# emma-mens/adam-compression

Hardware: AMD Instinct MI355X
Metric: grad elements/s per DGC step (HBM GB/s % of peak), 0.1% ratio, 1-8 GPUs (higher is better)
Workload: dtype f32

## Files before the change

adam-compression_amd/csrc/select.hip:

```cpp
#include <algorithm>
#include <cstdlib>
#include <cstring>
#include <cmath>
#include <vector>

#include "radix_select.hpp"
#include "introselect.hpp"

namespace dgc {

constexpr int kSeg = 1024;
constexpr int kCap = 64;
constexpr int kLstTile = 4;
__host__ __device__ __forceinline__ int64_t lcol(int64_t seg) {
    return (seg / kLstTile) * (kLstTile * kCap) + seg % kLstTile;
}
__host__ __device__ __forceinline__ int64_t lslot(int64_t seg, int64_t e, int64_t ntile) {
    (void)ntile;
    return lcol(seg) + e * kLstTile;
}
constexpr int kSegTiles = kSeg / (kWave * 4);
constexpr int kSuper = 4;
constexpr int kGroupSegs = 1024;
constexpr int kCountSegs = 4;
// ... 1330 lines not shown
    uint32_t vs[kSegTiles];
    load_segment(vec, d.n, ls, xs, vs);
    emit_segment_firstk(xs, vs, d, ls, base, limit, obase, t, o, mask_now);
}


constexpr int kEmitSegs = kGroupSegs / kEmitSplit;
constexpr int kEmitBatch = 16;
constexpr int kEmitShort = 16;
constexpr uint32_t kEmitSkip = 0xFFFFFFFFu;
static_assert(kCap == kWave, "wave-per-list emission needs kCap == wavefront width");

__device__ __forceinline__ void emit_body(const float* __restrict__ vec_flat, const SelWS& w, const EmitOut& oa,
                                          int64_t bx) {
    const int t = task(w, BT_GRP, (int)bx);
    const SelState* st = w.st + t;
    if (st->branch == DGC_BRANCH_RESAMPLE && st->rs_nth == 2) return;
    if (st->spec_emitted) return;
    const bool k5 = st->branch == DGC_BRANCH_RESAMPLE && st->rs_nth == 1;
    if (k5 && !oa.queue) return;
    EmitOut o = oa;
    if (!k5) o.queue = nullptr;
    const TDesc d = w.td[t];
    const bool defer_here = o.defer && !k5 && !d.tail;
    const float* vec = vec_flat + d.off;
    const int64_t lb = bx - w.bt[BT_GRP][t];
    const int64_t lg = lb / kEmitSplit;
    const int sub = (int)(lb % kEmitSplit);
    const int64_t g = d.grp0 + lg;
    const int64_t lseg0 = lg * kGroupSegs + (int64_t)sub * kEmitSegs;
    __shared__ uint32_t off_a[kEmitSegs], lcn[kEmitSegs];
    __shared__ uint64_t lds16[16];
    __shared__ long long obase_s;
    if (threadIdx.x < kWave) {
        const long long b = k5 ? 0 : out_base(w, t);
        if (threadIdx.x == 0) obase_s = b;
    }
    const long long limit = k5 ? st->n_cur : st->limit;
    const long long ga = w.grp_off[g];
    const float tc = st->t_cur;
    {
        const int jq = (int)threadIdx.x;
        const int64_t ls = lseg0 + jq;
        uint32_t ca = 0, lc = 0, pa = 0;
        if (ls < d.nseg) {
            const int64_t seg = d.seg0 + ls;
            ca = w.seg_cnt[seg];
            lc = lcnt_count(w.seg_lcnt[seg]);
        }
#pragma unroll
        for (int q = 0; q < kEmitSplit - 1; ++q) {
            if (q < sub) {
                const int64_t seg = d.seg0 + lg * kGroupSegs + (int64_t)q * kEmitSegs + threadIdx.x;
                pa += w.seg_cnt[seg];
            }
        }
        const bool short_list = ls < d.nseg && ca > 0 && lc <= (uint32_t)kEmitShort;
        float v[kEmitShort];
        uint16_t e[kEmitShort];
        if (short_list) {
            const int64_t ntile = ceil_div(w.nseg, (int64_t)kLstTile);
#pragma unroll
            for (int q = 0; q < kEmitShort; ++q)
                if ((uint32_t)q < lc) {
                    v[q] = w.lst_val[lslot(d.seg0 + ls, q, ntile)];
                    e[q] = w.lst_off[lslot(d.seg0 + ls, q, ntile)];
                }
        }
        uint64_t tot;
        const uint64_t ra = block_exclusive_scan(((uint64_t)pa << 32) | ca, lds16, &tot);
        const uint32_t oa = (uint32_t)(tot >> 32) + (uint32_t)ra;
        const bool work = ca > 0 && ga + oa < limit;
        if (defer_here && ls < d.nseg) w.seg_off[d.seg0 + ls] = oa;
        off_a[jq] = oa;
        lcn[jq] = (work && !short_list) ? lc : kEmitSkip;
        __syncthreads();
        if (work && short_list) {
            const long long ob0 = obase_s;
            long long pos = ga + oa;
#pragma unroll
            for (int j = 0; j < kEmitShort; ++j)
                if ((uint32_t)j < lc && fabsf(v[j]) >= tc) {
                    if (pos < limit) emit_one(o, d, ob0 + pos, ls * kSeg + e[j], v[j], !defer_here);
                    ++pos;
                }
        }
    }
    __syncthreads();
    const long long obase = obase_s;
    const int lane = threadIdx.x & 63, wv = threadIdx.x >> 6;
    const uint64_t lt = lanemask_lt();
    constexpr int kWaveSegs = kEmitSegs / (kEmitSegs / kWave);
    const int jw = wv * kWaveSegs;
    const uint32_t Lme = lane < kWaveSegs ? lcn[jw + lane] : kEmitSkip;
    uint64_t todo = __ballot(Lme != kEmitSkip && Lme <= (uint32_t)kCap);
    uint64_t spilled = __ballot(Lme != kEmitSkip && Lme > (uint32_t)kCap);
    for (int b0 = 0; b0 < kWaveSegs; b0 += kEmitBatch) {
        if (!((todo >> b0) & ((1ull << kEmitBatch) - 1))) continue;
        const int j0 = jw + b0;
        float x[kEmitBatch];
        uint32_t e[kEmitBatch];
#pragma unroll
        for (int q = 0; q < kEmitBatch; ++q) {
            const uint32_t L = lcn[j0 + q];
            x[q] = 0.f;
            e[q] = 0;
            if (L <= (uint32_t)kCap && (uint32_t)lane < L) {
                const int64_t slot = lslot(d.seg0 + lseg0 + j0 + q, lane, ceil_div(w.nseg, (int64_t)kLstTile));
                x[q] = w.lst_val[slot];
                e[q] = w.lst_off[slot];
            }
        }
#pragma unroll
        for (int q = 0; q < kEmitBatch; ++q) {
            const uint32_t L = lcn[j0 + q];
            if (L == kEmitSkip || L > (uint32_t)kCap) continue;
            const int64_t ls = lseg0 + j0 + q;
            const long long ba = ga + off_a[j0 + q];
            const bool sel = (uint32_t)lane < L && fabsf(x[q]) >= tc;
            const uint64_t m = __ballot(sel);
            const long long pos = ba + __popcll(m & lt);
            if (sel && pos < limit) emit_one(o, d, obase + pos, ls * kSeg + e[q], x[q], !defer_here);
        }
    }
    while (spilled) {
        const int j = jw + __builtin_ctzll(spilled);
        spilled &= spilled - 1;
        emit_reread_firstk(vec, d, lseg0 + j, ga + off_a[j], limit, obase, tc, o, !defer_here);
    }
}

__global__ void __launch_bounds__(kEmitSegs)
k_emit(const float* __restrict__ vec_flat, SelWS w, EmitOut oa) {
    emit_body(vec_flat, w, oa, blockIdx.x);
}

constexpr int kChainPhases = 3;
enum { CH_CLAIM = 0, CH_GATE = kChainPhases };
static_assert(32 + kChainPhases * 32 <= kChainOneWords, "SelWS::chain words");

template <bool ALIGNED>
__global__ void __launch_bounds__(kBlock)
k_chain_one(const float* __restrict__ vec_flat, SelWS w, SelCfg p) {
    uint32_t* cc = w.chain;
    __shared__ uint32_t s_u;
    bool open = false;
    for (int t = threadIdx.x; !open && t < w.T; t += blockDim.x) open = !w.st[t].done;
    if (!__syncthreads_or(open)) return;
    for (int ph = 0; ph < kChainPhases; ++ph) {
        bool any = false;
        for (int t = threadIdx.x; !any && t < w.T; t += blockDim.x) {
            const SelState& u = w.st[t];
            any = ph < 2 ? u.lower_pending != 0 : (u.active && u.t_cur >= u.t_list);
        }
        any = __syncthreads_or(any);
        if (threadIdx.x == 0) {
            uint32_t gate = __hip_atomic_load(&cc[CH_GATE + ph], __ATOMIC_RELAXED, __HIP_MEMORY_SCOPE_AGENT);
            if (gate == 0) {
                const uint32_t want = any ? 2u : 1u;
                const uint32_t prev = atomicCAS(&cc[CH_GATE + ph], 0u, want);
                gate = prev == 0u ? want : prev;
            }
            s_u = gate;
        }
        __syncthreads();
        if (s_u != 2u) continue;
        const int which = ph == 0 ? BT_SEG : ph == 1 ? BT_CAP4 : BT_CNT;
        const uint32_t nvb = (uint32_t)w.bt[which][w.T];
        uint32_t mine = 0;
        for (;;) {
            __syncthreads();
            if (threadIdx.x == 0) s_u = atomicAdd(&cc[CH_CLAIM + ph], 1u);
            __syncthreads();
            const uint32_t vb = s_u;
            if (vb >= nvb) break;
            if (ph == 0) lower_lists_body(vec_flat, w, p, vb);
            else if (ph == 1) lower_counts_body<ALIGNED>(vec_flat, w, p, vb);
            else count_lists_body(vec_flat, w, p, vb);
            ++mine;
        }
        chain_phase_end(reinterpret_cast<ChainPhase*>(cc + 32) + ph, mine, nvb);
    }
}



__device__ __forceinline__ void resample_set_block(const float* __restrict__ vec_flat, const SelWS& w,
                                                   const EmitOut& o, int bx, bool wait);

__device__ __forceinline__ bool emit_wide_part(const float* __restrict__ vec_flat, const SelWS& w, const EmitOut& oa,
                                               int bx) {
    const int t = task(w, BT_GRP, bx);
    const SelState* st = w.st + t;
    if (st->branch == DGC_BRANCH_RESAMPLE && st->rs_nth == 2) return false;
    if (st->spec_emitted) return false;
    const bool k5 = st->branch == DGC_BRANCH_RESAMPLE && st->rs_nth == 1;
    if (k5 && !oa.queue) return false;
    EmitOut o = oa;
    if (!k5) o.queue = nullptr;
    const TDesc d = w.td[t];
    const bool defer_here = o.defer && !k5 && !d.tail;
    const float* vec = vec_flat + d.off;
    const int64_t lb = (int64_t)bx - w.bt[BT_GRP][t];
    constexpr int split = kEmitSplit;
    const int64_t lg = lb / split;
    const int sub = (int)(lb % split);
    const int64_t g = d.grp0 + lg;
    const int64_t lseg0 = lg * kGroupSegs;
    __shared__ uint32_t off_a[kGroupSegs], lcn[kGroupSegs];
    __shared__ uint64_t lds16[16];
    __shared__ long long obase_s;
    if (threadIdx.x < kWave) {
        const long long b = k5 ? 0 : out_base(w, t);
        if (threadIdx.x == 0) obase_s = b;
    }
    const long long limit = k5 ? st->n_cur : st->limit;
    const long long ga = w.grp_off[g];
    {
        const int64_t ls = lseg0 + threadIdx.x;
        uint32_t ca = 0, lc = 0;
        if (ls < d.nseg) {
            const int64_t seg = d.seg0 + ls;
            ca = w.seg_cnt[seg];
            lc = lcnt_count(w.seg_lcnt[seg]);
        }
        uint64_t tot;
        const uint32_t oa = (uint32_t)block_exclusive_scan((uint64_t)ca, lds16, &tot);
        const bool work = ca > 0 && ga + oa < limit;
        if (defer_here && ls < d.nseg && (int)threadIdx.x / (kGroupSegs / split) == sub)
            w.seg_off[d.seg0 + ls] = oa;
        off_a[threadIdx.x] = oa;
        lcn[threadIdx.x] = work ? lc : kEmitSkip;
    }
    __syncthreads();
    ES_STAMP(1);
    const long long obase = obase_s;
    const float tc = st->t_cur;
    const int lane = threadIdx.x & 63, wv = threadIdx.x >> 6;
    const uint64_t lt = lanemask_lt();
    constexpr int wave_segs = kGroupSegs / split / (kGroupSegs / kWave);
    static_assert(wave_segs % kEmitBatch == 0, "whole batches per wave");
    const int jw = sub * (kGroupSegs / split) + wv * wave_segs;
    for (int j0 = jw; j0 < jw + wave_segs; j0 += kEmitBatch) {
        float x[kEmitBatch];
        uint32_t e[kEmitBatch];
#pragma unroll
        for (int q = 0; q < kEmitBatch; ++q) {
            const uint32_t L = lcn[j0 + q];
            x[q] = 0.f;
            e[q] = 0;
            if (L <= (uint32_t)kCap && (uint32_t)lane < L) {
                const int64_t slot = lslot(d.seg0 + lseg0 + j0 + q, lane, ceil_div(w.nseg, (int64_t)kLstTile));
                x[q] = w.lst_val[slot];
                e[q] = w.lst_off[slot];
            }
        }
        uint32_t spilled = 0;
#pragma unroll
        for (int q = 0; q < kEmitBatch; ++q) {
            const uint32_t L = lcn[j0 + q];
            if (L == kEmitSkip) continue;
            const int64_t ls = lseg0 + j0 + q;
            const long long ba = ga + off_a[j0 + q];
            if (L > (uint32_t)kCap) {
                spilled |= 1u << q;
                continue;
            }
            const bool sel = (uint32_t)lane < L && fabsf(x[q]) >= tc;
            const uint64_t m = __ballot(sel);
            const long long pos = ba + __popcll(m & lt);
            if (sel && pos < limit) emit_one(o, d, obase + pos, ls * kSeg + e[q], x[q], !defer_here);
        }
        while (spilled) {
            const int q = __builtin_ctz(spilled);
            spilled &= spilled - 1;
            emit_reread_firstk(vec, d, lseg0 + j0 + q, ga + off_a[j0 + q], limit, obase, tc, o, !defer_here);
        }
    }
    return k5;
}

template <bool SET>
__global__ void __launch_bounds__(kGroupSegs)
k_emit_wide_t(const float* __restrict__ vec_flat, SelWS w, EmitOut oa, EmitOut os, int32_t ngb) {
    const int bx = (int)blockIdx.x;
    ES_STAMP(0);
    if (SET && bx >= ngb) {
        resample_set_block(vec_flat, w, os, bx - ngb, true);
    } else if (emit_wide_part(vec_flat, w, oa, bx) && SET) {
        const int t = task(w, BT_GRP, bx);
        asm volatile("s_waitcnt vmcnt(0)" ::: "memory");
        __syncthreads();
        if (threadIdx.x == 0) {
            __builtin_amdgcn_fence(__ATOMIC_RELEASE, "agent");
            __hip_atomic_fetch_add(&w.setg[t].gathered, 1u, __ATOMIC_RELAXED, __HIP_MEMORY_SCOPE_AGENT);
        }
    }
    ES_STAMP(2);
}

constexpr unsigned long long kLbAgg = 1ull << 62, kLbPre = 1ull << 63, kLbVal = kLbAgg - 1;
constexpr int kLbSpin = 1 << 22;
constexpr int kCeStage = 2048;
#ifdef DGC_K5_PROF
__device__ unsigned long long g_ce_prof[2048][6];
#define CE_STAMP(i) do { if (threadIdx.x == 0 && lg < 2048) g_ce_prof[lg][i] = wall_clock64(); } while (0)
#else
#define CE_STAMP(i) do { } while (0)
#endif

__device__ __forceinline__ void count_emit_body(const float* __restrict__ vec_flat, const SelWS& w, const SelCfg& p,
                                                const EmitOut& o) {
    static_assert(kBlock * kCountSegs == kGroupSegs && kCountSegs == kLstTile, "k_count_emit layout");
    SelState* st = w.st;
    if (!st->active || !(st->t_cur >= st->t_list)) return;
    const TDesc d = w.td[0];
    const float* vec = vec_flat + d.off;
    const float tc = st->t_cur;
    const uint32_t tkey = abs_key(tc);
    const int tid = threadIdx.x, lane = tid & 63, wave = wave_id();
    __shared__ uint32_t lg_s;
    __shared__ int nspill;
    __shared__ int spill[kGroupSegs];
    __shared__ uint32_t spill_cnt[kGroupSegs];
    __shared__ uint64_t lds16[16];
    __shared__ unsigned long long prefix_s;
    __shared__ float stage_v[kCeStage];
    __shared__ uint32_t stage_i[kCeStage];
    if (tid == 0) {
        lg_s = atomicAdd(&st->ce_ticket, 1u);
        nspill = 0;
    }
    __syncthreads();
    const int64_t lg = lg_s;
    CE_STAMP(0);
    const int64_t ls0 = lg * kGroupSegs + kCountSegs * tid;
    const int64_t seg0 = d.seg0 + ls0;
    uint32_t n[kCountSegs], c[kCountSegs], lc[kCountSegs];
    if (ls0 + 3 < d.nseg) {
        const uint4 u = *reinterpret_cast<const uint4*>(w.seg_lcnt + seg0);
        lc[0] = u.x; lc[1] = u.y; lc[2] = u.z; lc[3] = u.w;
    } else {
#pragma unroll
        for (int q = 0; q < kCountSegs; ++q) lc[q] = ls0 + q < d.nseg ? w.seg_lcnt[seg0 + q] : 0u;
    }
#pragma unroll
    for (int q = 0; q < kCountSegs; ++q) {
        n[q] = ((lc[q] >> 16) << 16) <= tkey ? 0u : lcnt_count(lc[q]);
        c[q] = 0;
    }
    uint32_t nmax = 0;
#pragma unroll
    for (int q = 0; q < kCountSegs; ++q)
        if (n[q] <= (uint32_t)kCap) nmax = max(nmax, n[q]);
    constexpr int kFirst = 8;
    const int64_t ntile = ceil_div(w.nseg, (int64_t)kLstTile);
    const float* lv = w.lst_val;
    const uint16_t* lo = w.lst_off;
    float4 a[kFirst];
#pragma unroll
    for (int e = 0; e < kFirst; ++e)
        if ((uint32_t)e < nmax) a[e] = *reinterpret_cast<const float4*>(lv + lslot(seg0, e, ntile));
#pragma unroll
    for (int e = 0; e < kFirst; ++e) {
        const float x[4] = {a[e].x, a[e].y, a[e].z, a[e].w};
#pragma unroll
        for (int q = 0; q < kCountSegs; ++q) c[q] += (uint32_t)e < n[q] && n[q] <= (uint32_t)kCap && fabsf(x[q]) >= tc;
    }
    for (uint32_t e0 = kFirst; e0 < nmax; e0 += kFirst) {
        float4 b[kFirst];
#pragma unroll
        for (int e = 0; e < kFirst; ++e)
            if (e0 + e < nmax) b[e] = *reinterpret_cast<const float4*>(lv + lslot(seg0, e0 + e, ntile));
#pragma unroll
        for (int e = 0; e < kFirst; ++e) {
            if (e0 + e >= nmax) break;
            const float x[4] = {b[e].x, b[e].y, b[e].z, b[e].w};
#pragma unroll
            for (int q = 0; q < kCountSegs; ++q)
                c[q] += e0 + e < n[q] && n[q] <= (uint32_t)kCap && fabsf(x[q]) >= tc;
        }
    }
#pragma unroll
    for (int q = 0; q < kCountSegs; ++q)
        if (ls0 + q < d.nseg && n[q] > (uint32_t)kCap) spill[atomicAdd(&nspill, 1)] = kCountSegs * tid + q;
    __syncthreads();
    for (int i = wave; i < nspill; i += kBlock / kWave) {
        const int j = spill[i];
        const uint32_t cs = wave_count_segment(vec, d.n, lg * kGroupSegs + j, tc);
        if (lane == 0) spill_cnt[j] = cs;
    }
    __syncthreads();
#pragma unroll
    for (int q = 0; q < kCountSegs; ++q)
        if (ls0 + q < d.nseg && n[q] > (uint32_t)kCap) c[q] = spill_cnt[kCountSegs * tid + q];
    CE_STAMP(1);
    const uint32_t mine = c[0] + c[1] + c[2] + c[3];
    uint64_t total;
    const uint32_t tbase = (uint32_t)block_exclusive_scan((uint64_t)mine, lds16, &total);
    uint32_t off[kCountSegs];
    off[0] = tbase;
#pragma unroll
    for (int q = 1; q < kCountSegs; ++q) off[q] = off[q - 1] + c[q - 1];
#pragma unroll
    for (int q = 0; q < kCountSegs; ++q)
        if (ls0 + q < d.nseg) {
            w.seg_cnt[seg0 + q] = c[q];
            w.seg_off[seg0 + q] = off[q];
            if (n[q] > (uint32_t)kCap) spill_cnt[kCountSegs * tid + q] = off[q];
        }
    if (wave == 0) {
        unsigned long long* lb = w.grp_lb + d.grp0;
        if (lane == 0) {
            if (total) atomicAdd(&w.grp_cnt[d.grp0 + lg], (unsigned long long)total);
            __hip_atomic_store(&lb[lg], (lg == 0 ? kLbPre : kLbAgg) | total, __ATOMIC_RELAXED,
                               __HIP_MEMORY_SCOPE_AGENT);
        }
        unsigned long long prefix = 0;
        bool ok = true;
        int64_t j = lg - 1;
        int spin = 0;
        while (j >= 0) {
            const int64_t jj = j - lane;
            const unsigned long long v =
                jj >= 0 ? __hip_atomic_load(&lb[jj], __ATOMIC_RELAXED, __HIP_MEMORY_SCOPE_AGENT) : kLbPre;
            const uint64_t pre = __ballot((v & kLbPre) != 0), unready = __ballot(v == 0);
            const int first = pre ? __builtin_ctzll(pre) : kWave;
            const uint64_t need = first >= kWave - 1 ? ~0ull : ((2ull << first) - 1);
            if (unready & need) {
                if (++spin > kLbSpin) {
                    ok = false;
                    break;
                }
                __builtin_amdgcn_s_sleep(1);
                continue;
            }
            prefix += wave_sum(lane <= first ? (v & kLbVal) : 0ull);
            if (first < kWave) break;
            j -= kWave;
        }
        if (lane == 0) {
            if (lg > 0 && ok)
                __hip_atomic_store(&lb[lg], kLbPre | (prefix + total), __ATOMIC_RELAXED, __HIP_MEMORY_SCOPE_AGENT);
            if (!ok) atomicExch(&st->ce_fail, 1);
            prefix_s = ok ? prefix : ~0ull;
        }
    }
    __syncthreads();
    CE_STAMP(2);
    const unsigned long long P = prefix_s;
    const long long limit = d.k;
    const bool emit = P != ~0ull && (long long)P < limit;
    const bool staged = emit && nspill == 0 && total <= (uint64_t)kCeStage;
    if (emit) {
        for (uint32_t e0 = 0; e0 < nmax; e0 += kFirst) {
            if ((long long)(P + off[0]) >= limit) break;
            uint2 ob[kFirst];
            float4 vb[kFirst];
#pragma unroll
            for (int e = 0; e < kFirst; ++e)
                if (e0 + e < nmax) {
                    ob[e] = *reinterpret_cast<const uint2*>(lo + lslot(seg0, e0 + e, ntile));
                    vb[e] = *reinterpret_cast<const float4*>(lv + lslot(seg0, e0 + e, ntile));
                }
#pragma unroll
            for (int e = 0; e < kFirst; ++e) {
                if (e0 + e >= nmax) break;
                const float x[4] = {vb[e].x, vb[e].y, vb[e].z, vb[e].w};
                const uint32_t oo[4] = {ob[e].x & 0xFFFFu, ob[e].x >> 16, ob[e].y & 0xFFFFu, ob[e].y >> 16};
#pragma unroll
                for (int q = 0; q < kCountSegs; ++q)
                    if (e0 + e < n[q] && n[q] <= (uint32_t)kCap && fabsf(x[q]) >= tc) {
                        const uint32_t r = off[q];
                        if (staged) {
                            stage_v[r] = x[q];
                            stage_i[r] = (uint32_t)(kCountSegs * tid + q) * kSeg + oo[q];
                        } else if ((long long)(P + r) < limit) {
                            emit_one(o, d, (long long)(P + r), (ls0 + q) * kSeg + oo[q], x[q], false);
                        }
                        off[q] = r + 1;
                    }
            }
        }
    }
    if (emit && !staged)
        for (int i = wave; i < nspill; i += kBlock / kWave) {
            const int j = spill[i];
            emit_reread_firstk(vec, d, lg * kGroupSegs + j, (long long)(P + spill_cnt[j]), limit, 0, tc, o, false);
        }
    CE_STAMP(3);
    if (staged) {
        __syncthreads();
        const long long m = std::min<long long>((long long)total, limit - (long long)P);
        const int64_t gbase = lg * kGroupSegs * (int64_t)kSeg;
        for (long long i = tid; i < m; i += kBlock) {
            store_value(o.values, (long long)P + i, stage_v[i], o.vdtype);
            store_index(o.indices, (long long)P + i, d.idx_base + gbase + stage_i[i], o.idtype);
        }
    }
    CE_STAMP(4);
    if (last_block_arrival8(st->tk8, (uint32_t)lg, (uint32_t)(w.bt[BT_CNT][1] - w.bt[BT_CNT][0])))
        decide_tensor(w, p, 0, 1);
    CE_STAMP(5);
}

__global__ void __launch_bounds__(kBlock)
k_count_emit(const float* __restrict__ vec_flat, SelWS w, SelCfg p, EmitOut o) {
    count_emit_body(vec_flat, w, p, o);
}

template <bool ALIGNED>
__global__ void __launch_bounds__(kBlock)
k_count_emit_pass(const float* __restrict__ vec_flat, SelWS w, SelCfg p, EmitOut o, int which, int ncnt) {
    if ((int)blockIdx.x < ncnt)
        count_emit_body(vec_flat, w, p, o);
    else
        select_pass_body<ALIGNED>(vec_flat, w, which, p, (int64_t)blockIdx.x - ncnt);
}

struct FinishArgs {
    int64_t* count_out;
    dgc_select_info* info;
    float margin;
    int32_t defer, mask_mmt;
    int32_t on;
    int32_t* sink;
    uint32_t force;
    int64_t* order_out;
};

__device__ __forceinline__ void sel_finish_body(const SelWS& w, const FinishArgs& f) {
    int64_t* count_out = f.count_out;
    dgc_select_info* info = f.info;
    const float margin = f.margin;
    const int defer = f.defer, mask_mmt = f.mask_mmt;
    __shared__ unsigned long long total;
    __shared__ uint32_t broken, topk_order;
    if (threadIdx.x == 0) {
        total = 0;
        broken = 0;
        topk_order = 0;
    }
    __syncthreads();
    for (int t = threadIdx.x; t < w.T; t += blockDim.x) {
        SelState* st = w.st + t;
        struct {
            float t0, t_cur;
            int32_t branch, recounts, overflow, full_passes, list_spills, epoch, tie_rule, win_keys;
            long long n_cur, limit;
        } s;
        s.t0 = st->t0;
        s.t_cur = st->t_cur;
        s.branch = st->branch;
        s.recounts = st->recounts;
        s.overflow = st->overflow;
        s.full_passes = st->full_passes;
        s.list_spills = st->list_spills;
        s.epoch = st->epoch;
        s.tie_rule = st->tie_rule;
        s.win_keys = st->win_keys;
        s.n_cur = st->n_cur;
        s.limit = st->limit;
        const uint32_t wc = st->win_cnt[s.epoch & 1];
        const int64_t k = w.td[t].k;
        const bool tail = w.td[t].tail;
        const uint32_t status = w.nthg[t].status;
        float* spec = w.spec ? w.spec + kSpecWords * t : nullptr;
        const float used = spec ? spec[0] : __builtin_huge_valf();
        const float prev = spec ? spec[1] : __builtin_huge_valf();
        const uint32_t k5 = status | (s.branch == DGC_BRANCH_RESAMPLE ? f.force : 0u);
        if (k5 & DGC_K5_BROKEN) atomicOr(&broken, k5);
        if (s.branch == DGC_BRANCH_RESAMPLE && s.tie_rule == DGC_TIES_EXACT) atomicOr(&topk_order, 1u);
        const long long cnt = s.branch == DGC_BRANCH_RESAMPLE ? (long long)k : s.limit;
        atomicAdd(&total, (unsigned long long)cnt);
        st->epoch = s.epoch + 1;
        st->def_mode = (defer && s.branch != DGC_BRANCH_RESAMPLE && !tail && cnt > 0) ? 1 : 0;
        st->def_t = s.t_cur;
        st->def_limit = s.limit;
        st->def_mask_mmt = mask_mmt;
        if (info) {
            dgc_select_info& r = info[t];
            r.count = cnt;
            r.candidates = s.n_cur;
            r.threshold0 = s.t0;
            r.threshold = s.t_cur;
            r.branch = s.branch;
            r.recounts = s.recounts;
            r.overflow_segments = s.full_passes ? s.overflow : s.list_spills;
            r.full_passes = s.full_passes;
            r.tie_rule = s.tie_rule;
            r.window_keys = s.win_keys;
            r.k5_status = (int32_t)k5;
            r.list_threshold = used;
        }
        if (spec) {
            const float tc = s.t_cur;
            const bool finite = tc == tc && tc > 0.f && tc < __builtin_huge_valf();
            const float gr = fminf(fmaxf(2.f - prev / tc, 1.f), 1.5f);
            const float c0 = spec[4] < __builtin_huge_valf() ? spec[4] : fmaxf(margin, kSpecCeil0);
            const bool tried = used < __builtin_huge_valf() && tc > 0.f;
            const bool hit = tried && tc >= used;
            const float mcap = !tried ? c0
                                : hit ? fminf(c0 + kSpecCeilUp, fmaxf(margin, kSpecMarginMax))
                                      : fmaxf(c0 - kSpecCeilDown, margin);
            float m = margin;
            if (hit) m = fminf(fmaxf(1.05f * (used / tc), margin), mcap);
            spec[4] = mcap;
            spec[0] = finite ? tc * m * gr : __builtin_huge_valf();
            spec[1] = finite ? tc : __builtin_huge_valf();
            const float t0 = s.t0;
            const bool f0 = t0 == t0 && t0 > 0.f && t0 < __builtin_huge_valf();
            const float g0 = fminf(fmaxf(2.f - spec[3] / t0, 1.f), 1.5f);
            const float mw = wc > (uint32_t)kWinMax ? 0.985f : (s.win_keys > 0 ? 0.97f : 0.9f);
            spec[2] = f0 ? t0 * mw * g0 : __builtin_huge_valf();
            spec[3] = f0 ? t0 : __builtin_huge_valf();
        }
    }
    __syncthreads();
    if (threadIdx.x == 0 && count_out) *count_out = (int64_t)total;
    if (threadIdx.x == 0 && f.order_out) *f.order_out = topk_order ? 0 : (int64_t)DGC_ORDER_ASCENDING;
    if (threadIdx.x == 0 && broken && f.sink)
        __hip_atomic_store(f.sink, (int32_t)broken, __ATOMIC_RELAXED, __HIP_MEMORY_SCOPE_SYSTEM);
}

__global__ void k_sel_finish(SelWS w, FinishArgs f) { sel_finish_body(w, f); }

__global__ void __launch_bounds__(kBlock) k_emit_queue(const float* __restrict__ vec_flat, SelWS w, EmitOut o) {
    const int t = task(w, BT_QUEUE, blockIdx.x);
    const SelState* st = w.st + t;
    if (!(st->branch == DGC_BRANCH_RESAMPLE && st->rs_nth == 1)) return;
    const TDesc d = w.td[t];
    __shared__ long long obase_s;
    if (threadIdx.x < kWave) {
        const long long b = out_base(w, t);
        if (threadIdx.x == 0) obase_s = b;
    }
    __syncthreads();
    const int64_t q = ((int64_t)blockIdx.x - w.bt[BT_QUEUE][t]) * kQueuePerBlock + threadIdx.x;
    if (q >= d.k) return;
    const uint32_t j = (uint32_t)w.queue[d.cand_off + q];
    emit_one(o, d, obase_s + q, w.cand_idx[d.cand_off + j], w.cand_val[d.cand_off + j]);
}

constexpr int kHeapTop = 16383;
constexpr int kHeapChunk = kNthThreads * 4;
constexpr int kHeapSub = 5;
constexpr int kHeapKeyShift = 33;
constexpr uint64_t kHeapIdxMask = (1ull << kHeapKeyShift) - 1;
constexpr size_t kHeapSmemBytes = (size_t)(kHeapTop + 1 + kHeapChunk) * 8;
constexpr size_t kK5SmemBytes = kHeapSmemBytes > kNthSmemBytes ? kHeapSmemBytes : kNthSmemBytes;

__device__ __forceinline__ uint32_t hkey(uint64_t e) { return (uint32_t)(e >> kHeapKeyShift); }

struct HeapNodes {
    DGC_LDS uint64_t* l;
    DGC_GLB uint64_t* g;
    __device__ __forceinline__ uint64_t ld(int64_t i) const { return i < kHeapTop ? l[i] : g[i]; }
    __device__ __forceinline__ void st(int64_t i, uint64_t v) const {
        if (i < kHeapTop)
            l[i] = v;
        else
            g[i] = v;
    }
};

__device__ void heap_adjust1(const HeapNodes& h, int64_t hole, int64_t len, uint64_t v) {
    const int64_t top = hole;
    int64_t child = hole;
    while (child < (len - 1) / 2) {
        child = 2 * (child + 1);
        const uint64_t r = h.ld(child), l = h.ld(child - 1);
        uint64_t c = r;
        if (hkey(r) > hkey(l)) {
            child--;
            c = l;
        }
        h.st(hole, c);
        hole = child;
    }
    if ((len & 1) == 0 && child == (len - 2) / 2) {
        child = 2 * (child + 1);
        h.st(hole, h.ld(child - 1));
        hole = child - 1;
    }
    int64_t parent = (hole - 1) / 2;
    while (hole > top) {
        const uint64_t pv = h.ld(parent);
        if (!(hkey(pv) > hkey(v))) break;
        h.st(hole, pv);
        hole = parent;
        parent = (hole - 1) / 2;
    }
    h.st(hole, v);
}

__device__ __forceinline__ uint64_t readlane64(uint64_t x, int lane) {
    const uint32_t lo = (uint32_t)__builtin_amdgcn_readlane((int)(uint32_t)x, lane);
    const uint32_t hi = (uint32_t)__builtin_amdgcn_readlane((int)(uint32_t)(x >> 32), lane);
    return ((uint64_t)hi << 32) | lo;
}

__device__ uint64_t heap_replace_root(const HeapNodes& h, int64_t len, uint64_t v) {
    const int lane = threadIdx.x & 63;
    uint64_t pidx = 0, pval = 0;
    int m = 0;
    int64_t hole = 0;
    bool more = len > 1;
    while (more) {
        const int dl = 31 - __clz(lane + 2);
        const int64_t ol = (int64_t)(lane + 2) - (1ll << dl);
        const int64_t node = ((hole + 1) << dl) - 1 + ol;
        uint64_t val = 0;
        if (lane < 62 && node < len) val = h.ld(node);
        int64_t off = 0;
        for (int d = 1; d <= kHeapSub; ++d) {
            const int base = (1 << d) - 2;
            int64_t child;
            uint64_t cval;
            if (hole < (len - 1) / 2) {
                const uint64_t l = readlane64(val, base + (int)(2 * off));
                const uint64_t r = readlane64(val, base + (int)(2 * off) + 1);
                if (hkey(r) > hkey(l)) {
                    child = 2 * hole + 1;
                    cval = l;
                    off = 2 * off;
                } else {
                    child = 2 * hole + 2;
                    cval = r;
                    off = 2 * off + 1;
                }
            } else if ((len & 1) == 0 && hole == (len - 2) / 2) {
                child = 2 * hole + 1;
                cval = readlane64(val, base + (int)(2 * off));
                off = 2 * off;
                more = false;
            } else {
                more = false;
                break;
            }
            if (lane == m) {
                pidx = (uint64_t)child;
                pval = cval;
            }
            ++m;
            hole = child;
            if (!more) break;
        }
    }
    const uint64_t above = __ballot(lane < m && hkey(pval) > hkey(v));
    const int jm1 = above ? __builtin_ctzll(above) : m;
    const uint64_t up = (uint64_t)__shfl_up((long long)pidx, 1);
    const int64_t parent = lane == 0 ? 0 : (int64_t)up;
    if (lane < jm1)
        h.st(parent, pval);
    else if (lane == jm1)
        h.st(parent, v);
    __builtin_amdgcn_fence(__ATOMIC_RELEASE, "workgroup");
    __builtin_amdgcn_fence(__ATOMIC_ACQUIRE, "workgroup");
    return jm1 == 0 ? v : readlane64(pval, 0);
}

constexpr int kHeapAhead = 8;

__device__ __forceinline__ void heap_load(const float* vec, int64_t n, int64_t c0, bool al, float (&x)[4]) {
    const int64_t e0 = c0 + 4 * (int64_t)threadIdx.x;
    if (al && e0 + 3 < n) {
        const float4 v = *reinterpret_cast<const float4*>(vec + e0);
        x[0] = v.x;
        x[1] = v.y;
        x[2] = v.z;
        x[3] = v.w;
    } else {
#pragma unroll
        for (int j = 0; j < 4; ++j) x[j] = e0 + j < n ? vec[e0 + j] : 0.f;
    }
}

__device__ __forceinline__ uint32_t heap_cands(int64_t n, int64_t c0, float tc, const float (&x)[4]) {
    const int64_t e0 = c0 + 4 * (int64_t)threadIdx.x;
    uint32_t cm = 0;
#pragma unroll
    for (int j = 0; j < 4; ++j) cm |= (uint32_t)(e0 + j < n && fabsf(x[j]) >= tc) << j;
    return cm;
}

template <class F>
__device__ __forceinline__ int64_t heap_stream(const float* vec, int64_t n, int64_t c_begin, bool al, F&& f) {
    constexpr int64_t kBatch = (int64_t)kHeapAhead * kHeapChunk;
    float xa[kHeapAhead][4], xb[kHeapAhead][4];
#pragma unroll
    for (int u = 0; u < kHeapAhead; ++u) heap_load(vec, n, c_begin + u * kHeapChunk, al, xa[u]);
    for (int64_t b0 = c_begin; b0 < n; b0 += kBatch) {
#pragma unroll
        for (int u = 0; u < kHeapAhead; ++u) heap_load(vec, n, b0 + kBatch + u * kHeapChunk, al, xb[u]);
#pragma unroll
        for (int u = 0; u < kHeapAhead; ++u) {
            const int64_t c0 = b0 + u * kHeapChunk;
            if (c0 >= n) return c0;
            if (!f(c0, xa[u])) return c0;
        }
#pragma unroll
        for (int u = 0; u < kHeapAhead; ++u)
#pragma unroll
            for (int j = 0; j < 4; ++j) xa[u][j] = xb[u][j];
    }
    return n;
// ... 1426 lines not shown
```

Before: 293.5 billion.

## Capture selected entries during count pass and stage them while awaiting lookback prefix

During the count pass, each thread now also loads the list offsets and records up to 15 above-threshold values with their tags in per-thread LDS slots. When every entry fits (no spills, no capture overflow, total within the stage buffer), waves other than the lookback wave write the staged output while wave 0 spins on the decoupled lookback. This removes the second read of the list values and offsets in the emit phase and hides staging behind the prefix wait. In exchange it adds LDS (the spill arrays are aliased into stage_i), extra offset loads in the count loop, and register pressure that could lower occupancy.

```diff
diff --git a/adam-compression_amd/csrc/select.hip b/adam-compression_amd/csrc/select.hip
--- a/adam-compression_amd/csrc/select.hip
+++ b/adam-compression_amd/csrc/select.hip
@@ -1656,11 +1656,15 @@
 constexpr unsigned long long kLbAgg = 1ull << 62, kLbPre = 1ull << 63, kLbVal = kLbAgg - 1;
 constexpr int kLbSpin = 1 << 22;
 constexpr int kCeStage = 2048;
+constexpr int kCeCap = 15;
 #ifdef DGC_K5_PROF
-__device__ unsigned long long g_ce_prof[2048][6];
-#define CE_STAMP(i) do { if (threadIdx.x == 0 && lg < 2048) g_ce_prof[lg][i] = wall_clock64(); } while (0)
+__device__ unsigned long long g_ce_prof[2048][7];
+#define CE_STAMP_T(i, t) do { if (threadIdx.x == (t) && lg < 2048) g_ce_prof[lg][i] = wall_clock64(); } while (0)
+#define CE_STAMP(i) CE_STAMP_T(i, 0)
+#define CE_STAMP_W1(i) CE_STAMP_T(i, kWave)
 #else
 #define CE_STAMP(i) do { } while (0)
+#define CE_STAMP_W1(i) do { } while (0)
 #endif
 
 __device__ __forceinline__ void count_emit_body(const float* __restrict__ vec_flat, const SelWS& w, const SelCfg& p,
@@ -1674,16 +1678,21 @@
     const uint32_t tkey = abs_key(tc);
     const int tid = threadIdx.x, lane = tid & 63, wave = wave_id();
     __shared__ uint32_t lg_s;
-    __shared__ int nspill;
-    __shared__ int spill[kGroupSegs];
-    __shared__ uint32_t spill_cnt[kGroupSegs];
+    __shared__ int nspill, ncapover;
     __shared__ uint64_t lds16[16];
     __shared__ unsigned long long prefix_s;
     __shared__ float stage_v[kCeStage];
     __shared__ uint32_t stage_i[kCeStage];
+    static_assert(2 * kGroupSegs <= kCeStage, "spill records fit in stage_i");
+    int* const spill = reinterpret_cast<int*>(stage_i);
+    uint32_t* const spill_cnt = stage_i + kGroupSegs;
+    static_assert(kSeg <= 1024 && kCountSegs <= 4, "a capture's tag: list << 10 | offset");
+    __shared__ float cap_v[kCeCap][kBlock];
+    __shared__ uint16_t cap_t[kCeCap][kBlock];
     if (tid == 0) {
         lg_s = atomicAdd(&st->ce_ticket, 1u);
         nspill = 0;
+        ncapover = 0;
     }
     __syncthreads();
     const int64_t lg = lg_s;
@@ -1711,30 +1720,59 @@
     const int64_t ntile = ceil_div(w.nseg, (int64_t)kLstTile);
     const float* lv = w.lst_val;
     const uint16_t* lo = w.lst_off;
+    uint32_t ncap = 0;
+    const auto capture = [&](float x, uint32_t o16, int q) {
+        if (ncap < (uint32_t)kCeCap) {
+            cap_v[ncap][tid] = x;
+            cap_t[ncap][tid] = (uint16_t)((uint32_t)q << 10 | o16);
+        }
+        ++ncap;
+    };
+    static_assert(kFirst % 2 == 0 && kCap % 2 == 0, "offsets load in pairs of entries");
     float4 a[kFirst];
+    uint4 ao[kFirst / 2];
 #pragma unroll
     for (int e = 0; e < kFirst; ++e)
-        if ((uint32_t)e < nmax) a[e] = *reinterpret_cast<const float4*>(lv + lslot(seg0, e, ntile));
+        if ((uint32_t)e < nmax) {
+            if (e % 2 == 0) ao[e / 2] = *reinterpret_cast<const uint4*>(lo + lslot(seg0, e, ntile));
+            a[e] = *reinterpret_cast<const float4*>(lv + lslot(seg0, e, ntile));
+        }
 #pragma unroll
     for (int e = 0; e < kFirst; ++e) {
         const float x[4] = {a[e].x, a[e].y, a[e].z, a[e].w};
-#pragma unroll
-        for (int q = 0; q < kCountSegs; ++q) c[q] += (uint32_t)e < n[q] && n[q] <= (uint32_t)kCap && fabsf(x[q]) >= tc;
+        const uint32_t o01 = e % 2 ? ao[e / 2].z : ao[e / 2].x, o23 = e % 2 ? ao[e / 2].w : ao[e / 2].y;
+        const uint32_t oo[4] = {o01 & 0xFFFFu, o01 >> 16, o23 & 0xFFFFu, o23 >> 16};
+#pragma unroll
+        for (int q = 0; q < kCountSegs; ++q)
+            if ((uint32_t)e < n[q] && n[q] <= (uint32_t)kCap && fabsf(x[q]) >= tc) {
+                ++c[q];
+                capture(x[q], oo[q], q);
+            }
     }
     for (uint32_t e0 = kFirst; e0 < nmax; e0 += kFirst) {
         float4 b[kFirst];
+        uint4 bo[kFirst / 2];
 #pragma unroll
         for (int e = 0; e < kFirst; ++e)
-            if (e0 + e < nmax) b[e] = *reinterpret_cast<const float4*>(lv + lslot(seg0, e0 + e, ntile));
+            if (e0 + e < nmax) {
+                if (e % 2 == 0) bo[e / 2] = *reinterpret_cast<const uint4*>(lo + lslot(seg0, e0 + e, ntile));
+                b[e] = *reinterpret_cast<const float4*>(lv + lslot(seg0, e0 + e, ntile));
+            }
 #pragma unroll
         for (int e = 0; e < kFirst; ++e) {
             if (e0 + e >= nmax) break;
             const float x[4] = {b[e].x, b[e].y, b[e].z, b[e].w};
+            const uint32_t o01 = e % 2 ? bo[e / 2].z : bo[e / 2].x, o23 = e % 2 ? bo[e / 2].w : bo[e / 2].y;
+            const uint32_t oo[4] = {o01 & 0xFFFFu, o01 >> 16, o23 & 0xFFFFu, o23 >> 16};
 #pragma unroll
             for (int q = 0; q < kCountSegs; ++q)
-                c[q] += e0 + e < n[q] && n[q] <= (uint32_t)kCap && fabsf(x[q]) >= tc;
-        }
-    }
+                if (e0 + e < n[q] && n[q] <= (uint32_t)kCap && fabsf(x[q]) >= tc) {
+                    ++c[q];
+                    capture(x[q], oo[q], q);
+                }
+        }
+    }
+    if (ncap > (uint32_t)kCeCap) atomicOr(&ncapover, 1);
 #pragma unroll
     for (int q = 0; q < kCountSegs; ++q)
         if (ls0 + q < d.nseg && n[q] > (uint32_t)kCap) spill[atomicAdd(&nspill, 1)] = kCountSegs * tid + q;
@@ -1763,6 +1801,23 @@
             w.seg_off[seg0 + q] = off[q];
             if (n[q] > (uint32_t)kCap) spill_cnt[kCountSegs * tid + q] = off[q];
         }
+    CE_STAMP(2);
+    const auto all_captured = [&]() { return nspill == 0 && ncapover == 0 && total <= (uint64_t)kCeStage; };
+    const auto stage_captures = [&]() {
+        uint32_t r0 = off[0], r1 = off[1], r2 = off[2], r3 = off[3];
+        for (uint32_t i = 0; i < min(ncap, (uint32_t)kCeCap); ++i) {
+            const uint32_t t = cap_t[i][tid];
+            const uint32_t q = t >> 10;
+            const uint32_t r = q == 0 ? r0 : q == 1 ? r1 : q == 2 ? r2 : r3;
+            stage_v[r] = cap_v[i][tid];
+            stage_i[r] = (uint32_t)(kCountSegs * tid) * kSeg + t;
+            r0 += q == 0;
+            r1 += q == 1;
+            r2 += q == 2;
+            r3 += q == 3;
+        }
+    };
+    bool captured;
     if (wave == 0) {
         unsigned long long* lb = w.grp_lb + d.grp0;
         if (lane == 0) {
@@ -1770,6 +1825,7 @@
             __hip_atomic_store(&lb[lg], (lg == 0 ? kLbPre : kLbAgg) | total, __ATOMIC_RELAXED,
                                __HIP_MEMORY_SCOPE_AGENT);
         }
+        captured = all_captured();
         unsigned long long prefix = 0;
         bool ok = true;
         int64_t j = lg - 1;
@@ -1799,14 +1855,19 @@
             if (!ok) atomicExch(&st->ce_fail, 1);
             prefix_s = ok ? prefix : ~0ull;
         }
+        if (captured) stage_captures();
+    } else {
+        captured = all_captured();
+        if (captured) stage_captures();
+        CE_STAMP_W1(3);
     }
     __syncthreads();
-    CE_STAMP(2);
+    CE_STAMP(4);
     const unsigned long long P = prefix_s;
     const long long limit = d.k;
     const bool emit = P != ~0ull && (long long)P < limit;
     const bool staged = emit && nspill == 0 && total <= (uint64_t)kCeStage;
-    if (emit) {
+    if (emit && !captured) {
         for (uint32_t e0 = 0; e0 < nmax; e0 += kFirst) {
             if ((long long)(P + off[0]) >= limit) break;
             uint2 ob[kFirst];
@@ -1842,9 +1903,8 @@
             const int j = spill[i];
             emit_reread_firstk(vec, d, lg * kGroupSegs + j, (long long)(P + spill_cnt[j]), limit, 0, tc, o, false);
         }
-    CE_STAMP(3);
     if (staged) {
-        __syncthreads();
+        if (!captured) __syncthreads();
         const long long m = std::min<long long>((long long)total, limit - (long long)P);
         const int64_t gbase = lg * kGroupSegs * (int64_t)kSeg;
         for (long long i = tid; i < m; i += kBlock) {
@@ -1852,10 +1912,10 @@
             store_index(o.indices, (long long)P + i, d.idx_base + gbase + stage_i[i], o.idtype);
         }
     }
-    CE_STAMP(4);
+    CE_STAMP(5);
     if (last_block_arrival8(st->tk8, (uint32_t)lg, (uint32_t)(w.bt[BT_CNT][1] - w.bt[BT_CNT][0])))
         decide_tensor(w, p, 0, 1);
-    CE_STAMP(5);
+    CE_STAMP(6);
 }
 
 __global__ void __launch_bounds__(kBlock)
```

Result: slower. 283.6 billion (-3.4%).
